# GuildOfWeavers/distaff

Hardware: AMD Instinct MI355X
Metric: trace_cells_per_sec (higher is better)
Workload: dtype u128 (prime field 2^128-45*2^40+1, 4x u32 limbs)

## Files before the change

distaff_amd/csrc/air_kernel.h:

```cpp
#pragma once
#include "ctx.h"
#include <type_traits>

#ifndef AIR_THREADS
#define AIR_THREADS 128
#endif
#ifdef AIR_CONVOY
#define AIR_SYNC() __builtin_amdgcn_s_barrier()
#else
#define AIR_SYNC()
#endif
#ifndef AIR_WAVES_PER_SIMD
#define AIR_WAVES_PER_SIMD 2
#endif
constexpr int air_waves_per_simd(int sd, int slcap, int sect) {
    (void)sd; (void)slcap; (void)sect;
#ifdef AIR_WAVES_FORCE
    return AIR_WAVES_FORCE;
#else
    return AIR_WAVES_PER_SIMD;
#endif
}

struct AirConsts { fe sponge_mds[16], sponge_inv_mds[16], hasher_mds[36], hasher_inv_mds[36]; };
// ... 114 lines not shown
        if constexpr (I == ST_AUX0) return is_bin(o[0]);
        else if constexpr (I == ST_AUX1) return is_bin(o[1]);
        else if constexpr (I == 0) return fe_sub(nw[0], fe_mul(o[0], o[1]));
        else return L(1);
    }
    else if constexpr (OP == 0x0B) {
        if constexpr (I == ST_AUX0) return is_bin(o[0]);
        else if constexpr (I == ST_AUX1) return is_bin(o[1]);
        else if constexpr (I == 0) return fe_sub(nw[0], fe_sub(fe_add(o[0], o[1]), fe_mul(o[0], o[1])));
        else return L(1);
    }
    else if constexpr (OP == 0x0C) { if constexpr (I == 0) return fe_sub(fe_one(), fe_mul(nw[0], o[0])); else return C(); }
    else if constexpr (OP == 0x0D) { if constexpr (I == 0) return fe_add(nw[0], o[0]); else return C(); }
    else if constexpr (OP == 0x0E) {
        if constexpr (I == ST_AUX0) return is_bin(o[0]);
        else if constexpr (I == 0) return fe_sub(nw[0], bnot(o[0]));
        else return C();
    }
    else if constexpr (OP == 0x10) return R(1);
    else if constexpr (OP == 0x11) return R(2);
    else if constexpr (OP == 0x12) { if constexpr (I == 0) return fe_sub(nw[0], o[0]); else return R(1); }
    else if constexpr (OP == 0x13) { if constexpr (I < 2) return fe_sub(nw[i], o[i]); else return R(2); }
    else if constexpr (OP == 0x14) { if constexpr (I < 4) return fe_sub(nw[i], o[i]); else return R(4); }
    else if constexpr (OP == 0x15) { if constexpr (I < 2) return nw[i]; else return R(2); }
    else if constexpr (OP == 0x18) { if constexpr (I == 0) return fe_add(fe_sub(nw[0], o[1]), fe_sub(nw[1], o[0])); else return C(); }
    else if constexpr (OP == 0x19) { if constexpr (I < 4) return fe_sub(nw[i], o[i ^ 2]); else return C(); }
    else if constexpr (OP == 0x1A) return fe_sub(nw[i], o[i ^ 4]);
    else if constexpr (OP == 0x1B) { if constexpr (I < 4) return fe_sub(nw[i], o[(i + 3) & 3]); else return C(); }
    else if constexpr (OP == 0x1C) return fe_sub(nw[i], o[(i + 7) & 7]);
    else if constexpr (OP == 0x1D) {
        if constexpr (I == 0) return is_bin(nw[0]);
        else if constexpr (I == 1) return nw[1];
        else if constexpr (I == 2) return fe_sub(nw[2], fe_double(o[2]));
        else if constexpr (I == 3) return fe_sub(nw[3], fe_add(o[3], fe_mul(nw[0], o[2])));
        else return C();
    }
    else return fe_zero();
}

#define AG_LOW(c, b) (1u << ((c) * 4 + (b)))
#define AG_LOW0 0x00Fu
#define AG_LOW1 0x0F0u
#define AG_PUSH 0x100u
#define AG_CMP 0x200u
#define AG_RESCR 0x400u
#define AG_KEEP 0x800u
#define AG_HIGH 0xF00u
#define AG_DEEP 0x1000u
#define AG_STACK_ALL 0x1FFFu
#define AF_FIRST 1
#define AF_LAST 2
#define AF_EV_IN 4
#define AF_EV_OUT 8

struct StDesc { int kind, j; };
template <int SDK, bool DEEP>
constexpr StDesc st_desc(int op, int I) {
    const bool o4_zero = SDK != 0 && SDK <= 4;
    if (I >= 8) {
        if ((op == 0x0A || op == 0x0B)) return StDesc{5, I == ST_AUX0 ? 100 : 101};
        if ((op == 0x06 || op == 0x07) && o4_zero) return StDesc{0, 0};
        return StDesc{5, -1};
    }
    const int i = I;
    auto diff = [&](int j) { return (SDK != 0 && j >= SDK) ? StDesc{4, 0} : StDesc{1, j}; };
    auto rdiff = [&](int j) { return (SDK != 0 && j >= SDK) ? StDesc{3, 0} : StDesc{2, j}; };
    auto L = [&](int num) { return i + num < 8 ? diff(i + num) : (DEEP ? StDesc{5, -1} : StDesc{3, 0}); };
    auto R = [&](int num) { return diff(i - num < 0 ? 0 : i - num); };
    switch (op) {
        case 0x00: return L(1);
        case 0x01: return L(2);
        case 0x02: return i == 0 ? StDesc{5, -1} : L(2);
        case 0x03: return L(1);
        case 0x04: return L(4);
        case 0x05: return i == 0 ? StDesc{5, -1} : L(2);
        case 0x06: return i < 2 ? (o4_zero ? rdiff(i + 2) : StDesc{5, -1}) : L(4);
        case 0x07: return i < 4 ? (o4_zero ? rdiff(i) : StDesc{5, -1}) : L(2);
        case 0x08: case 0x0B: return i == 0 ? StDesc{5, -1} : L(1);
        case 0x09: case 0x0A: return i == 0 ? StDesc{5, 102} : L(1);
        case 0x0C: case 0x0D: case 0x0E: return i == 0 ? StDesc{5, -1} : diff(i);
        case 0x10: return R(1);
        case 0x11: return R(2);
        case 0x12: return i == 0 ? rdiff(0) : R(1);
        case 0x13: return i < 2 ? rdiff(i) : R(2);
        case 0x14: return i < 4 ? rdiff(i) : R(4);
        case 0x15: return i < 2 ? StDesc{3, 0} : R(2);
        case 0x18: return i == 0 ? StDesc{5, -1} : diff(i);
        case 0x19: return i < 4 ? rdiff(i ^ 2) : diff(i);
        case 0x1A: return rdiff(i ^ 4);
        case 0x1B: return i < 4 ? rdiff((i + 3) & 3) : diff(i);
        case 0x1C: return rdiff((i + 7) & 7);
        case 0x1D: return i == 1 ? StDesc{3, 0} : (i < 4 ? StDesc{5, -1} : diff(i));
        default: return StDesc{0, 0};
    }
}
struct StMerge { int n; int kind[4], j[4], lead[4]; int sgn[4][4]; };
template <int BASE, int I, int SDK, bool DEEP>
constexpr StMerge st_merge() {
    StMerge m{};
    for (int a = 0; a < 4; a++) {
        const StDesc d = st_desc<SDK, DEEP>(BASE + a, I);
        bool has = false;
        switch (a) { case 0: has = st_has<BASE, I>(); break; case 1: has = st_has<BASE + 1, I>(); break; case 2: has = st_has<BASE + 2, I>(); break; default: has = st_has<BASE + 3, I>(); }
        if (!has || d.kind == 0) continue;
        const int cls = d.kind == 5 ? 5 : (d.kind <= 2 ? 1 : 3);
        const int sign = (d.kind == 2 || d.kind == 4) ? -1 : 1;
// ... 54 lines not shown
                constexpr int base = 4 * b + 16 * c;
                if constexpr ((GROUPS & AG_LOW(c, b)) != 0) {
                    static constexpr StMerge M = st_merge<base, I, SDK, DEEP>();
                    if constexpr (M.n > 0) {
                        fe_acc inner; fe_acc_zero(inner);
                        static_for_air<0, M.n>([&](auto e_) {
                            constexpr int e = decltype(e_)::value;
                            fe cf = (base == 0 && M.lead[e] == 0) ? lo0h : lo2[M.lead[e]];
                            static_for_air<0, 4>([&](auto a_) {
                                constexpr int a = decltype(a_)::value;
                                if constexpr (a != M.lead[e] && M.sgn[e][a] != 0) {
                                    const fe other = (base == 0 && a == 0) ? lo0h : lo2[a];
                                    cf = M.sgn[e][a] > 0 ? fe_add(cf, other) : fe_sub(cf, other);
                                }
                            });
                            constexpr int ii = I < 8 ? I : 0;
                            fe term;
                            if constexpr (M.kind[e] == 1) term = fe_sub(s.o[M.j[e]], s.nw[ii]);
                            else if constexpr (M.kind[e] == 2) term = fe_sub(s.nw[ii], s.o[M.j[e]]);
                            else if constexpr (M.kind[e] == 3) term = s.nw[ii];
                            else if constexpr (M.kind[e] == 4) term = fe_neg(s.nw[ii]);
                            else term = st_term<base + M.lead[e], I>(s);
                            fe_acc_mac(inner, cf, term);
                        });
                        fe_acc_mac(middle, mid[b], fe_acc_reduce(inner));
                    }
                }
            });
            fe_acc_mac(outer, top[c], fe_acc_reduce(middle));
        }
    });
    if constexpr ((GROUPS & AG_HIGH) != 0) st_high_degree<I, GROUPS>(outer, s, h);
    return fe_acc_reduce(outer);
}

template <uint32_t ACC_MASK>
struct Acc {
    fe_acc res_acc;
    fe_acc adj_acc[6];
    fe res, adj[6];
    bool nonzero;
    const fe* tc; uint32_t nc;
    __device__ __forceinline__ void emit(uint32_t cidx, int slot, const fe& d) {
        nonzero |= !fe_is_zero(d);
        fe_acc_mac(res_acc, d, tc[cidx]);
        if ((ACC_MASK >> slot) & 1u) fe_acc_mac(adj_acc[slot], d, tc[nc + cidx]);
        else adj[slot] = fe_add(adj[slot], fe_mul(d, tc[nc + cidx]));
    }
};

template <int CL, int LL, int SD, int SLCAP, int SECT, uint32_t GROUPS, int FLAGS>
__global__ void __launch_bounds__(AIR_THREADS, air_waves_per_simd(SD, SLCAP, SECT)) air_kernel(AirArgs a) {
    constexpr bool FIRST = (FLAGS & AF_FIRST) != 0, LAST = (FLAGS & AF_LAST) != 0, EV_IN = (FLAGS & AF_EV_IN) != 0, EV_OUT = (FLAGS & AF_EV_OUT) != 0;
    constexpr int SL = SD ? (SD > 8 ? SD : 8) : SLCAP;
    constexpr bool DEEP = SD == 0 && SLCAP == 12;
    const int cl = (int)a.cl, ll = (int)a.ll;
    const int sl = SD ? SL : (int)a.sl;
    const int sd = SD ? SD : (int)a.stack_depth;
    const fe* c_sponge_mds = a.consts->sponge_mds; const fe* c_sponge_inv_mds = a.consts->sponge_inv_mds;
    const fe* c_hasher_mds = a.consts->hasher_mds; const fe* c_hasher_inv_mds = a.consts->hasher_inv_mds;
    const size_t k = (size_t)blockIdx.x * AIR_THREADS + threadIdx.x;
    if (k >= a.n) return;
    const uint32_t ql = blockIdx.y;
    const uint32_t qg = a.q0 + ql;
    const uint32_t jl = ql * a.coset_step;
    const size_t kn = (k + 1 == a.n) ? 0 : k + 1;
    const fe* cur_p = a.lde + (size_t)jl * a.n + k;
    const fe* nxt_p = a.lde + (size_t)jl * a.n + kn;
    const size_t cs = a.col_stride;
#define CUR(c) cur_p[(size_t)(c) * cs]
#define NXT(c) nxt_p[(size_t)(c) * cs]

    const uint64_t nmask = ((uint64_t)1 << a.log_N) - 1;
    const uint64_t gi = ((uint64_t)k << a.log_b) + (uint64_t)qg * a.coset_step;
    const uint32_t step = (uint32_t)(((uint64_t)k << 3) + qg);
    const uint64_t n64 = a.n;

    const fe c_opc = CUR(0), n_opc = NXT(0);
    fe c_sp[4], n_sp[4], cf[3], ld[5], hd[2], n_cf[3];
#pragma unroll
    for (int i = 0; i < 4; i++) { c_sp[i] = CUR(1 + i); n_sp[i] = NXT(1 + i); }
#pragma unroll
    for (int i = 0; i < 3; i++) { cf[i] = CUR(5 + i); n_cf[i] = NXT(5 + i); }
#pragma unroll
    for (int i = 0; i < 5; i++) ld[i] = CUR(8 + i);
#pragma unroll
    for (int i = 0; i < 2; i++) hd[i] = CUR(13 + i);
    fe c_ctx[CL], n_ctx[CL], c_lp[LL], n_lp[LL], o[SL], nw[SL];
    {
        uint32_t col = 15;
#pragma unroll
        for (int i = 0; i < CL; i++) { bool on = (uint32_t)i < a.ctx_depth; c_ctx[i] = on ? CUR(col + i) : fe_zero(); n_ctx[i] = on ? NXT(col + i) : fe_zero(); }
        col += a.ctx_depth;
#pragma unroll
        for (int i = 0; i < LL; i++) { bool on = (uint32_t)i < a.loop_depth; c_lp[i] = on ? CUR(col + i) : fe_zero(); n_lp[i] = on ? NXT(col + i) : fe_zero(); }
        col += a.loop_depth;
#pragma unroll
        for (int i = 0; i < SL; i++) { bool on = i < sd; o[i] = on ? CUR(col + i) : fe_zero(); nw[i] = on ? NXT(col + i) : fe_zero(); }
    }

    if constexpr ((SECT & 1) != 0) {
        const fe xp = dpow(a, (gi * (6 * n64 + 2)) & nmask);
        const fe one = fe_one();
#pragma unroll 1
        for (int pass = 0; pass < 2; pass++) {
            const fe* cc = a.coef + pass * 94;
            fe_acc R, A; fe_acc_zero(R); fe_acc_zero(A);
            auto term = [&](const fe& v, uint32_t idx) { fe_acc_mac(R, v, cc[idx]); fe_acc_mac(A, v, cc[idx + 1]); };
            term(pass ? fe_sub(c_opc, a.op_count) : c_opc, 0);
            if (pass == 0) { for (int i = 0; i < 4; i++) term(c_sp[i], 2 + 2 * i); }
            else { for (int i = 0; i < 2; i++) term(fe_sub(c_sp[i], a.program_hash[i]), 2 + 2 * i); }
            for (int i = 0; i < 3; i++) term(pass ? fe_sub(cf[i], one) : cf[i], 10 + 2 * i);
            for (int i = 0; i < 5; i++) term(pass ? fe_sub(ld[i], one) : ld[i], 16 + 2 * i);
            for (int i = 0; i < 2; i++) term(pass ? fe_sub(hd[i], one) : hd[i], 26 + 2 * i);
            for (int i = 0; i < CL; i++) if (i < cl) term(c_ctx[i], 30 + 2 * i);
            for (int i = 0; i < LL; i++) if (i < ll) term(c_lp[i], 62 + 2 * i);
            const uint32_t nio = pass ? a.num_outputs : a.num_inputs;
#pragma unroll
            for (int i = 0; i < 8; i++) if ((uint32_t)i < nio) term(fe_sub(o[i], pass ? a.outputs[i] : a.inputs[i]), 78 + 2 * i);
            const fe adj = fe_acc_reduce(A);
            fe_acc_mac(R, adj, xp);
            a.out[((size_t)pass * gridDim.y + ql) * a.n + k] = fe_acc_reduce(R);
        }
    }

    AIR_SYNC();
    fe cff[8], hdf[4], begin_flag, noop_flag, n_void, assert_flag;
    fe lo2[4], mid[4], top[2];
    {
        fe n0 = bnot(cf[0]), n1 = bnot(cf[1]), n2 = bnot(cf[2]);
        fe t0 = fe_mul(n0, n1), t1 = fe_mul(cf[0], n1), t2 = fe_mul(n0, cf[1]), t3 = fe_mul(cf[0], cf[1]);
        cff[0] = fe_mul(t0, n2); cff[1] = fe_mul(t1, n2); cff[2] = fe_mul(t2, n2); cff[3] = fe_mul(t3, n2);
        cff[4] = fe_mul(t0, cf[2]); cff[5] = fe_mul(t1, cf[2]); cff[6] = fe_mul(t2, cf[2]); cff[7] = fe_mul(t3, cf[2]);
        n_void = fe_mul(fe_mul(n_cf[0], n_cf[1]), n_cf[2]);
        fe l0 = bnot(ld[0]), l1 = bnot(ld[1]), l2 = bnot(ld[2]), l3 = bnot(ld[3]);
        lo2[0] = fe_mul(l0, l1); lo2[1] = fe_mul(ld[0], l1);
        lo2[2] = fe_mul(l0, cf[1]);
        lo2[3] = fe_mul(ld[0], ld[1]);
        mid[0] = fe_mul(l2, l3); mid[1] = fe_mul(ld[2], l3); mid[2] = fe_mul(l2, ld[3]); mid[3] = fe_mul(ld[2], ld[3]);
        top[0] = bnot(ld[4]); top[1] = ld[4];
        fe h0 = bnot(hd[0]), h1 = bnot(hd[1]);
        hdf[0] = fe_mul(h0, h1); hdf[1] = fe_mul(hd[0], h1); hdf[2] = fe_mul(h0, hd[1]); hdf[3] = fe_mul(hd[0], hd[1]);
    }
    auto LDF = [&](int idx) { return fe_mul(fe_mul(lo2[idx & 3], mid[(idx >> 2) & 3]), top[idx >> 4]); };
    {
        fe ld0 = LDF(0);
        begin_flag = fe_mul(ld0, hdf[0]);
        noop_flag = fe_mul(LDF(31), hdf[3]);
        hdf[0] = fe_mul(hdf[0], ld[0]);
        assert_flag = fe_mul(ld0, hd[0]);
    }

    AIR_SYNC();
    const fe* per = a.periodic + (size_t)(step & 127u) * AIR_PERIODIC_STRIDE;
    constexpr uint32_t ACC_MASK = !(SD != 0 || SLCAP == 8 || DEEP) ? 0u : ((SECT & 2) ? 0x01u : 0x3Fu);
    Acc<ACC_MASK> acc;
#pragma unroll
    for (int i = 0; i < 6; i++) if ((ACC_MASK >> i) & 1u) fe_acc_zero(acc.adj_acc[i]);
    fe_acc_zero(acc.res_acc); acc.res = fe_zero(); acc.nonzero = false; acc.tc = a.tc; acc.nc = 20 + cl + ll + 2 + sd;
#pragma unroll
    for (int i = 0; i < 6; i++) acc.adj[i] = fe_zero();
    const size_t pstride = (size_t)gridDim.y * a.n, pidx = (size_t)ql * a.n + k;

    if constexpr ((SECT & 2) != 0) {
        fe cf_sum = fe_add(fe_add(cf[0], cf[1]), cf[2]);
        fe ld_prod = fe_mul(fe_mul(fe_mul(ld[0], ld[1]), fe_mul(ld[2], ld[3])), ld[4]);
        fe hd_prod = fe_mul(hd[0], hd[1]);
#pragma unroll
        for (int i = 0; i < 3; i++) acc.emit(i, 0, is_bin(cf[i]));
#pragma unroll
        for (int i = 0; i < 5; i++) acc.emit(3 + i, 0, is_bin(ld[i]));
#pragma unroll
        for (int i = 0; i < 2; i++) acc.emit(8 + i, 0, is_bin(hd[i]));
        const fe is_hacc = cff[0];
        fe hacc_tr = fe_mul(fe_add(c_opc, fe_one()), is_hacc);
        fe rest_tr = fe_mul(c_opc, bnot(is_hacc));
        acc.emit(10, 1, fe_sub(fe_add(hacc_tr, rest_tr), n_opc));
        acc.emit(11, 5, fe_mul(c_opc, fe_mul(bnot(ld_prod), bnot(hd_prod))));
        acc.emit(12, 5, fe_mul(cf_sum, bnot(fe_mul(ld_prod, hd_prod))));
        acc.emit(13, 3, fe_mul(cff[7], bnot(n_void)));
        fe prefix = fe_add(fe_add(cff[1], cff[4]), fe_add(cff[5], cff[6]));
        fe v = fe_mul(prefix, per[21]);
        v = fe_add(v, fe_mul(fe_add(cff[2], cff[3]), per[20]));
        v = fe_add(v, fe_mul(hdf[0], per[22]));
        acc.emit(14, 2, v);
    }

    if constexpr ((SECT & 4) != 0) {
        fe sp[4];
        const fe f_begin = cff[1], f_tend = cff[2], f_fend = cff[3], f_loop = cff[4], f_wrap = cff[5], f_break = cff[6], f_void = cff[7];
        {
            fe os[4], ns[4];
#pragma unroll
            for (int i = 0; i < 4; i++) os[i] = fe_cube(fe_add(c_sp[i], per[i]));
            matmul<4>(os, c_sponge_mds);
            fe op_code = hd[1];
            op_code = fe_add(fe_double(op_code), hd[0]);
            op_code = fe_add(fe_double(op_code), ld[4]);
            op_code = fe_add(fe_double(op_code), ld[3]);
            op_code = fe_add(fe_double(op_code), ld[2]);
            op_code = fe_add(fe_double(op_code), ld[1]);
            op_code = fe_add(fe_double(op_code), ld[0]);
            os[0] = fe_add(os[0], op_code);
            os[1] = fe_add(os[1], fe_mul(nw[0], hdf[0]));
#pragma unroll
            for (int i = 0; i < 4; i++) ns[i] = n_sp[i];
            matmul<4>(ns, c_sponge_inv_mds);
#pragma unroll
            for (int i = 0; i < 4; i++) ns[i] = fe_sub(fe_cube(ns[i]), per[4 + i]);
            const fe clr = fe_add(fe_add(f_begin, f_loop), f_wrap);
            const fe cpy = fe_add(f_break, f_void);
            const fe tf = fe_add(f_tend, f_fend);
            const fe xf[4] = {tf, f_tend, f_fend, tf};
            const fe xv[4] = {fe_sub(c_ctx[0], n_sp[0]), fe_sub(c_sp[0], n_sp[1]), fe_sub(c_sp[0], n_sp[2]), n_sp[3]};
#pragma unroll
            for (int i = 0; i < 4; i++) {
                fe_acc A; fe_acc_zero(A);
                fe_acc_mac(A, cff[0], fe_sub(os[i], ns[i]));
                fe_acc_mac(A, clr, n_sp[i]);
                fe_acc_mac(A, cpy, fe_sub(c_sp[i], n_sp[i]));
                fe_acc_mac(A, xf[i], xv[i]);
                sp[i] = fe_acc_reduce(A);
            }
        }
        acc.emit(15, 3, sp[0]); acc.emit(16, 4, sp[1]); acc.emit(17, 3, sp[2]); acc.emit(18, 3, sp[3]);
    }
    if constexpr ((SECT & 128) != 0) {
        const fe f_begin = cff[1], f_tend = cff[2], f_fend = cff[3], f_loop = cff[4], f_wrap = cff[5], f_break = cff[6], f_void = cff[7];
        acc.emit(19, 2, fe_mul(fe_add(f_wrap, f_break), fe_sub(c_sp[0], c_lp[0])));
        const fe push = fe_add(f_begin, f_loop), pop = fe_add(f_tend, f_fend), ccpy = fe_add(fe_add(f_wrap, f_break), f_void);
        const fe lcpy = fe_add(fe_add(fe_add(f_begin, f_tend), fe_add(f_fend, f_wrap)), f_void);
        if constexpr (CL <= 2 && LL <= 1) {
#pragma unroll
            for (int i = 0; i < CL; i++) {
                if (i >= cl) break;
                fe_acc A; fe_acc_zero(A);
                fe_acc_mac(A, push, fe_sub(i == 0 ? c_sp[0] : c_ctx[i - 1 < 0 ? 0 : i - 1], n_ctx[i]));
                fe_acc_mac(A, pop, i + 1 < cl ? fe_sub(c_ctx[i + 1 < CL ? i + 1 : 0], n_ctx[i]) : n_ctx[i]);
                fe_acc_mac(A, ccpy, fe_sub(c_ctx[i], n_ctx[i]));
                const fe v = fe_acc_reduce(A);
                acc.emit(20 + i, 2, v);
            }
#pragma unroll
            for (int i = 0; i < LL; i++) {
                if (i >= ll) break;
                fe v = fe_mul(lcpy, fe_sub(c_lp[i], n_lp[i]));
                if (i >= 1) v = fe_add(v, fe_mul(f_loop, fe_sub(c_lp[i - 1 < 0 ? 0 : i - 1], n_lp[i])));
                v = fe_add(v, fe_mul(f_break, i + 1 < ll ? fe_sub(c_lp[i + 1 < LL ? i + 1 : 0], n_lp[i]) : n_lp[i]));
                acc.emit(20 + cl + i, 2, v);
            }
        } else {
            auto ctx_cur = [&](int i) { return (uint32_t)i < a.ctx_depth ? CUR(15 + i) : fe_zero(); };
            auto ctx_nxt = [&](int i) { return (uint32_t)i < a.ctx_depth ? NXT(15 + i) : fe_zero(); };
            const uint32_t lcol = 15 + a.ctx_depth;
            auto lp_cur = [&](int i) { return (uint32_t)i < a.loop_depth ? CUR(lcol + i) : fe_zero(); };
            auto lp_nxt = [&](int i) { return (uint32_t)i < a.loop_depth ? NXT(lcol + i) : fe_zero(); };
#pragma unroll 1
            for (int i = 0; i < cl; i++) {
                const fe ni = ctx_nxt(i);
                fe_acc A; fe_acc_zero(A);
                fe_acc_mac(A, push, fe_sub(i == 0 ? c_sp[0] : ctx_cur(i - 1), ni));
                fe_acc_mac(A, pop, i + 1 < cl ? fe_sub(ctx_cur(i + 1), ni) : ni);
                fe_acc_mac(A, ccpy, fe_sub(ctx_cur(i), ni));
                acc.emit(20 + i, 2, fe_acc_reduce(A));
// ... 189 lines not shown
            f = hdf[2];
            fe os[6], ns[6];
#pragma unroll
            for (int i = 0; i < 6; i++) os[i] = fe_cube(fe_add(o[i], per[8 + i]));
            matmul<6>(os, c_hasher_mds);
#pragma unroll
            for (int i = 0; i < 6; i++) ns[i] = nw[i];
            matmul<6>(ns, c_hasher_inv_mds);
#pragma unroll
            for (int i = 0; i < 6; i++) ns[i] = fe_sub(fe_cube(ns[i]), per[14 + i]);
#pragma unroll
            for (int i = 0; i < 6; i++) agg(i, f, fe_sub(ns[i], os[i]));
            copy_from(6, f);
        }
        }

        const uint32_t sbase = 20 + cl + ll;
        if constexpr ((SECT & 40) != 0) { acc.emit(sbase, 4, aux0); acc.emit(sbase + 1, 4, aux1); }
#pragma unroll
        for (int i = 0; i < SLR; i++) if (i < sd) acc.emit(sbase + 2 + i, 4, ev[i]);
    }
    if constexpr (DEEP && (GROUPS & AG_DEEP) != 0) {
        {
            const uint32_t sbase = 20 + cl + ll;
            const fe lo_all = fe_add(fe_add(lo2[0], lo2[1]), fe_add(lo2[2], lo2[3]));
            fe fl1, fl2, fl4, fr1, fr2, fr4, fcp;
            { fe_acc A; fe_acc_zero(A); fe_acc_mac(A, mid[0], lo2[3]); fe_acc_mac(A, mid[2], lo_all); fl1 = fe_add(fe_mul(top[0], fe_acc_reduce(A)), assert_flag); }
            { fe_acc A; fe_acc_zero(A); fe_acc_mac(A, mid[0], fe_add(lo2[1], lo2[2])); fe_acc_mac(A, mid[1], fe_add(lo2[1], lo2[3])); fl2 = fe_mul(top[0], fe_acc_reduce(A)); }
            fl4 = fe_mul(top[0], fe_mul(mid[1], fe_add(lo2[0], lo2[2])));
            fr1 = fe_add(fe_mul(top[1], fe_mul(mid[0], fe_add(lo2[0], lo2[2]))), hdf[0]);
            { fe_acc A; fe_acc_zero(A); fe_acc_mac(A, mid[0], fe_add(lo2[1], lo2[3])); fe_acc_mac(A, mid[1], lo2[1]); fr2 = fe_mul(top[1], fe_acc_reduce(A)); }
            fr4 = fe_mul(top[1], fe_mul(mid[1], lo2[0]));
            {
                fe_acc A; fe_acc_zero(A); fe_acc_mac(A, mid[2], lo_all); fe_acc_mac(A, mid[3], fe_add(lo2[0], lo2[1]));
                fe_acc B; fe_acc_zero(B); fe_acc_mac(B, top[1], fe_acc_reduce(A)); fe_acc_mac(B, top[0], fe_mul(mid[3], fe_add(fe_add(lo2[0], lo2[1]), lo2[2])));
                fcp = fe_add(fe_add(fe_acc_reduce(B), fe_add(hdf[1], hdf[2])), fe_add(begin_flag, noop_flag));
            }
            const uint32_t scol = 15 + a.ctx_depth + a.loop_depth;
#pragma unroll 1
            for (int i = 8; i < sd; i++) {
                const fe ni = NXT(scol + i);
                auto item = [&](int j) { return CUR(scol + j); };
                auto left = [&](int num) { return i + num < sl ? fe_sub(item(i + num), ni) : ni; };
                fe_acc A; fe_acc_zero(A);
                fe_acc_mac(A, fcp, fe_sub(item(i), ni));
                fe_acc_mac(A, fr1, fe_sub(item(i - 1), ni)); fe_acc_mac(A, fr2, fe_sub(item(i - 2), ni)); fe_acc_mac(A, fr4, fe_sub(item(i - 4), ni));
                fe_acc_mac(A, fl1, left(1)); fe_acc_mac(A, fl2, left(2)); fe_acc_mac(A, fl4, left(4));
                acc.emit(sbase + 2 + i, 4, fe_acc_reduce(A));
            }
        }
    }

    if constexpr (SECT == 1) return;
    const bool on_trace = (qg == 0);
    if (on_trace && k + 1 != a.n && acc.nonzero) atomicMin(a.bad_step, (unsigned long long)k);
    acc.res = fe_acc_reduce(acc.res_acc);
    constexpr bool EMITS_STACK = (SECT & 120) != 0 || (GROUPS & AG_DEEP) != 0 || ((GROUPS & AG_STACK_ALL) != 0 && !EV_OUT);
    constexpr uint32_t USED = ((SECT & 2) ? 0x2Fu : 0u) | ((SECT & 4) ? 0x18u : 0u) | ((SECT & 128) ? 0x04u : 0u) | (EMITS_STACK ? 0x10u : 0u);
#pragma unroll
    for (int i = 0; i < 6; i++) if (((ACC_MASK & USED) >> i) & 1u) acc.adj[i] = fe_add(acc.adj[i], fe_acc_reduce(acc.adj_acc[i]));
    if constexpr (!FIRST) {
        acc.res = fe_add(acc.res, a.partial[pidx]);
#pragma unroll
        for (int i = 0; i < 6; i++) if (LAST || ((USED >> i) & 1u)) acc.adj[i] = fe_add(acc.adj[i], a.partial[(size_t)(i + 1) * pstride + pidx]);
    }
    if constexpr (!LAST) {
        a.partial[pidx] = acc.res;
#pragma unroll
        for (int i = 0; i < 6; i++) if (FIRST || ((USED >> i) & 1u)) a.partial[(size_t)(i + 1) * pstride + pidx] = acc.adj[i];
        return;
    }
    fe t;
    if (on_trace && k + 1 != a.n) {
        t = fe_zero();
    } else {
        const uint32_t degs[6] = {2, 3, 4, 6, 7, 8};
        fe_acc T; fe_acc_zero(T);
        fe_acc_add(T, acc.res);
#pragma unroll
        for (int g = 0; g < 6; g++) {
            uint64_t p = 8 * n64 - 1 - (n64 - 1) * degs[g];
            fe_acc_mac(T, acc.adj[g], dpow(a, (gi * p) & nmask));
        }
        t = fe_acc_reduce(T);
    }
    a.out[((size_t)2 * gridDim.y + ql) * a.n + k] = t;
#undef CUR
#undef NXT
}


template <int CL, int LL, int SD, int SLCAP, int SECT, uint32_t GROUPS, int FLAGS>
static void launch_air(dst_ctx* c, const AirArgs& a, uint32_t Q) {
    dim3 g((unsigned)((c->n + AIR_THREADS - 1) / AIR_THREADS), Q);
    static char name[64];
    if (!name[0]) snprintf(name, sizeof(name), "air_kernel<%d,%d,%d,%d,%d,%u,%d>", CL, LL, SD, SLCAP, SECT, (unsigned)GROUPS, FLAGS);
    constexpr int NS = SD == 4 ? 6 : 10;
    const double units = c->W + ((FLAGS & AF_FIRST) ? 0 : 7) + ((FLAGS & AF_LAST) ? 1 : 7) + ((SECT & 1) ? 2 : 0) + ((FLAGS & AF_EV_IN) ? NS : 0) + ((FLAGS & AF_EV_OUT) ? NS : 0);
    { KScope ks_(c, name, 16.0 * c->n * Q * units, true); hipLaunchKernelGGL((air_kernel<CL, LL, SD, SLCAP, SECT, GROUPS, FLAGS>), g, dim3(AIR_THREADS), 0, c->stream, a); }
}
void air_launch_sd4(dst_ctx* c, const AirArgs& a, uint32_t Q);
void air_launch_small(dst_ctx* c, const AirArgs& a, uint32_t Q);
void air_launch_deep(dst_ctx* c, const AirArgs& a, uint32_t Q);
void air_launch_generic(dst_ctx* c, const AirArgs& a, uint32_t Q);
```

distaff_amd/csrc/ctx.h:

```cpp
#pragma once
#include <hip/hip_runtime.h>
#include <stdint.h>
#include <string.h>
#include <memory>
#include <string>
#include <map>
#include <vector>
#include "fe.h"
#include "../../include/distaff_hip.h"

struct __attribute__((aligned(16))) digest { uint32_t w[8]; };
#define AIR_PERIODIC_STRIDE 29

#ifndef NTT_TW4_PAIRS
#define NTT_TW4_PAIRS 0
#endif
#if NTT_TW4_PAIRS
typedef fe_tw tw4_t;
#else
typedef fe tw4_t;
#endif

#define DST_MAX_FRI_LAYERS 24

struct dst_switch_def { const char* name; bool product; const char* values; const char* what; };
static const dst_switch_def DST_SWITCHES[] = {
    {"DISTAFF_SHARD_DEBUG",        true,  "1",               "stderr line per tree exchange on rank 0; communicators record the order of their collectives (dst_comm_trace)"},
    {"DISTAFF_SHARD_TREE_GATHER",  true,  "1",               "sharded Merkle trees: all-gather of all boundary nodes + upper levels repeated on every rank (BASELINE north_star's all-gather-only form) instead of the k-range all-to-all"},
    {"DISTAFF_SHARD_NO_OVERLAP",   true,  "1",               "sharded prover: every collective on the context's main stream (no second stream / events) also on a stream-ordered transport"},
    {"DISTAFF_COMM_TIMEOUT_S",     true,  "seconds",         "communicators: limit of every host wait behind a collective (default 60; <= 0: none); on expiry the rank aborts the communicator and returns DST_ERR_COMM (dst_comm_set_timeout changes it per handle)"},
    {"DISTAFF_LOCAL_TRANSPORT",    true,  "blocking",        "in-process transport (dst_comm_init_local, dst_prove_sharded_local): drain every rank's stream around each collective instead of the stream-ordered form (events between the ranks' streams, nothing waited for)"},
    {"DISTAFF_TMP_REGS",           true,  "4..W",            "registers per transform launch = size of the staging array (default: as many as 12 GiB hold, at most W)"},
    {"DISTAFF_AIR",                false, "small|deep|generic", "force a more general constraint-kernel instance set than the trace shape needs (generic = per-operation formulation)"},
    {"DISTAFF_BOUNDARY",           false, "eval",            "boundary combinations by evaluation on the 8n domain (the reference's route) instead of coefficient form"},
    {"DISTAFF_COMBINE",            false, "steps",           "combine_polys / DEEP composition as the reference's sequence of whole-array steps instead of the fused passes"},
    {"DISTAFF_NTT",                false, "pre|3pass|reg|lds", "force a transform plan family"},
    {"DISTAFF_NTT_SHAPE",          false, "a,b",             "three-pass plans: log2 of the first two pass lengths"},
    {"DISTAFF_NTT_ORDER",          false, "0",               "first pass of an extension in coset-slow block order"},
    {"DISTAFF_NTT_WAVES",          false, "4|8",             "force the 512- or 1024-lane instances of the LDS passes"},
    {"DISTAFF_NTT_FIXED",          false, "0",               "use the any-shape instances where a shape-compiled one exists"},
    {"DISTAFF_NTT_DIF",            false, "0|1|2",           "first pass of an extension: coset DIT (0), pre-scale + DIF (1), DIT with last-stage twiddles from global memory (2)"},
    {"DISTAFF_NTT_DEBUG",          false, "1",               "print the occupancy of every transform launch shape once"},
    {"DISTAFF_LDE_BATCH",          false, "cols,cosets",     "registers x cosets per transform launch"},
    {"DISTAFF_FOLD8_DFT",          false, "0",               "8n-coefficient extensions without the fused fold + 8-point step"},
    {"DISTAFF_TRACE_BUFFER",       false, "1",               "give the trace its own buffer instead of coset 0 of the extension"},
    {"DISTAFF_MERKLE_LEVEL2_LOG",  false, "k",               "build two tree levels per launch from 2^k grandparents per launch on (default 2^19)"},
    {"DISTAFF_MERKLE_LEVELS",      false, "1",               "one launch per tree level"},
    {"DISTAFF_SYN_DIV_TABLES",     false, "1",               "synthetic division by power tables + scan instead of the blocked form"},
    {"DISTAFF_FRI_TAIL",           false, "0",               "no single-launch tail: every FRI layer by its own launches (the tail otherwise starts at the first layer of at most 2^13 elements)"},
    {"DISTAFF_FRI_CHAIN",          false, "0",               "FRI commit phase with a root read-back and a host draw per layer"},
    {"DISTAFF_FRI_REPLICATE_LOG",  false, "k",               "sharded prover: replicate FRI layers from 2^k elements on (default 2^17)"},
    {"DISTAFF_SHARD_FORCE_OVERLAP", false, "1",              "sharded prover: the two-stream choreography of a stream-ordered transport over a blocking one"},
    {"DISTAFF_TEST_STALL_COLLECTIVE", false, "k|k@r",        "communicators: fault injection -- before device collective number k (of rank r only) a kernel holds the stream until the communicator is aborted"},
};
enum : size_t {
    HS_WEIGHTS = 0,
    HS_WEIGHTS_BYTES = (4 * 128 + 4) * 16,
    HS_DEEP = 32768,
    HS_DEEP_HALF = 2048,
    HS_FRI_ROOTS = 40960,
    HS_FRI_SLOTS = 45056,
    HS_FRI_SLOT_BYTES = 800,
    HS_AIR_FLAG = 65536 - 64,
    HS_DRAWS = 65536,
    HS_DRAWS_BYTES = (344 + 160) * 16,
    HS_COMPOSE = 65536 + 8192,
    HS_COMPOSE_BYTES = 516 * 16,
    HS_STATUS = 65536 + 8192 + 8320,
    HS_STATUS_SLOTS = 32,
    HS_TREE_READBACK = 65536 + 8192 + 8320 + 2048,
    HS_TAIL_ROOTS = HS_TREE_READBACK + 1024,
    HS_POW = HS_TAIL_ROOTS + 1024,
    HS_TOTAL = 131072
};
static_assert(HS_WEIGHTS + HS_WEIGHTS_BYTES <= HS_DEEP, "boundary weights overlap the DEEP values");
static_assert(HS_DEEP_HALF >= 128 * 16 && HS_DEEP + 2 * HS_DEEP_HALF <= HS_FRI_ROOTS, "DEEP values: W <= 128 registers");
static_assert(HS_FRI_ROOTS + DST_MAX_FRI_LAYERS * 32 <= HS_FRI_SLOTS, "FRI roots overlap the layer slots");
static_assert(8 * 96 + 32 <= HS_FRI_SLOT_BYTES && HS_FRI_SLOTS + DST_MAX_FRI_LAYERS * HS_FRI_SLOT_BYTES <= HS_AIR_FLAG, "FRI layer slots: G <= 8 ranks, DST_MAX_FRI_LAYERS layers");
static_assert(HS_DRAWS + HS_DRAWS_BYTES <= HS_COMPOSE && HS_COMPOSE + HS_COMPOSE_BYTES <= HS_STATUS && HS_STATUS + HS_STATUS_SLOTS * 64 <= HS_TOTAL, "upload regions overlap");
static_assert(HS_STATUS_SLOTS >= 2 + DST_MAX_FRI_LAYERS, "one status slot per tree exchange of a proof");
static_assert(HS_STATUS + HS_STATUS_SLOTS * 64 <= HS_TREE_READBACK && 8 * 96 + 32 <= 1024 && DST_MAX_FRI_LAYERS * 32 <= 1024 && HS_POW + 64 <= HS_TOTAL, "read-back regions overlap");

#ifdef DISTAFF_TEST_HOOKS
#define DST_TEST_HOOKS 1
#else
#define DST_TEST_HOOKS 0
// ... 124 lines not shown
    bool have_trace = false, committed = false, constraints_done = false, composed = false;
    hipStream_t upload_stream = nullptr;
    std::vector<hipEvent_t> upload_done;
    std::vector<size_t> upload_bounds;
    bool upload_pending = false;
    bool trace_owned_only = false;
    bool ceval_inverted = false;
    hipStream_t comm_stream = nullptr;
    std::vector<hipEvent_t> comm_events;
    uint8_t* d_status = nullptr;
    double phase_ms[9] = {0};
    double shard_ms[2] = {0, 0};
    uint32_t shard_trees = 0;
    struct dst_comm* wait_comm = nullptr;
    hipEvent_t sh_ev[8] = {nullptr};
    struct CollEv { hipEvent_t e0, e1; int kind; };
    std::vector<CollEv> coll_ev;
    size_t coll_used = 0;
    double exchange_ms[8] = {0};

    int profile = 0;
    struct KEvent { hipEvent_t e0, e1; std::string name; double bytes, mads; };
    std::vector<KEvent> kpending;
    std::vector<hipEvent_t> event_pool;
    struct KStat { uint64_t launches = 0; double ms = 0, bytes = 0, mads = 0; };
    std::map<std::string, KStat> kstats;
};

struct KScope {
    dst_ctx* c; bool on;
    dst_ctx::KEvent ev;
    KScope(dst_ctx* ctx, const char* name, double bytes, bool heavy = false, double mads = 0.0) : c(ctx), on(ctx->profile == 1 || (ctx->profile == 2 && heavy)) {
        if (!on) return;
        ev.name = name; ev.bytes = bytes; ev.mads = mads;
        if (c->event_pool.size() >= 2) { ev.e0 = c->event_pool.back(); c->event_pool.pop_back(); ev.e1 = c->event_pool.back(); c->event_pool.pop_back(); }
        else if (hipEventCreate(&ev.e0) != hipSuccess || hipEventCreate(&ev.e1) != hipSuccess) { on = false; return; }
        (void)hipEventRecord(ev.e0, c->stream);
    }
    ~KScope() { if (on) { (void)hipEventRecord(ev.e1, c->stream); c->kpending.push_back(ev); } }
};

#define HIP_TRY(ctx, expr)                                                                          \
    do {                                                                                            \
        hipError_t _e = (expr);                                                                     \
        if (_e != hipSuccess) {                                                                     \
            (ctx)->err = std::string(#expr) + ": " + hipGetErrorString(_e);                          \
            return DST_ERR_HIP;                                                                     \
        }                                                                                           \
    } while (0)

int ctx_sync(dst_ctx* c, const char* what);
#define CTX_SYNC(ctx, what) do { const int _r = ctx_sync((ctx), (what)); if (_r) return _r; } while (0)

inline bool dst_internal_boundary_by_evaluation(const dst_ctx* c) { return DST_TEST_HOOKS && c->sw_is("DISTAFF_BOUNDARY", "eval"); }
inline bool dst_internal_combine_by_steps(const dst_ctx* c) { return DST_TEST_HOOKS && (c->sw_is("DISTAFF_COMBINE", "steps") || dst_internal_boundary_by_evaluation(c)); }
inline bool fri_tail_starts_at(const dst_ctx* c, int d) {
    if (d < 1 || d >= c->num_fri_layers || c->fri_size[d] > ((size_t)1 << 13)) return false;
    const char* e = c->sw("DISTAFF_FRI_TAIL");
    return !(e && e[0] == '0');
}
int k_ntt_init(dst_ctx* c);
void k_intt_columns(dst_ctx* c, const fe* src, size_t src_stride, fe* dst, size_t ncols);
void k_lde_columns(dst_ctx* c, const fe* polys, fe* lde, size_t ncols);
void k_lde_fold8(dst_ctx* c, const fe* poly8n, fe* out);
void k_intt8_cosets(dst_ctx* c, fe* vals , fe* out8n, fe* work);
void k_coset_to_natural_len(dst_ctx* c, const fe* src, size_t cosets, size_t len, fe* dst);
void k_fri_leaves_at(dst_ctx* c, const fe* e, digest* leaves, size_t R);
void k_fri_fold_at(dst_ctx* c, const fe* e, fe* out, size_t R, int layer, fe special_x, const fe* alpha_dev = nullptr);
void k_trace_leaves(dst_ctx* c);
void k_merkle(dst_ctx* c, const digest* leaves, digest* nodes, size_t count, size_t stop_count);
void k_constraint_tree(dst_ctx* c);
void k_fri_leaves_layer0(dst_ctx* c);
void k_fri_leaves(dst_ctx* c, int layer);
int k_eval_constraints(dst_ctx* c, const fe* coeffs_dev, const fe* tc_dev, int64_t* bad_step, bool defer_check = false);
int k_constraint_check(dst_ctx* c, int64_t* bad_step);
void k_syn_div(dst_ctx* c, fe* a, size_t len, fe b);
void k_syn_div_batch(dst_ctx* c, fe* const* a, const fe* b, int count, size_t len);
void k_syn_div_compose(dst_ctx* c, const fe* a, fe* out, size_t len, fe b, const fe* t, size_t tn, size_t inc, fe k1, fe k2, fe k3);
void k_combine_fused(dst_ctx* c, const fe* work, const fe* q4, size_t q_stride, fe* cpoly);
void k_syn_div_expanded(dst_ctx* c, const fe* a, fe* out, size_t len, size_t degree, fe exception);
void k_horner(dst_ctx* c, const fe* polys, size_t ncols, size_t len, fe x, fe* out_dev);
void k_lincomb(dst_ctx* c, const fe* cols, size_t ncols, size_t len, const fe* coeffs_dev, fe* out);
void k_lincomb2(dst_ctx* c, const fe* cols, size_t ncols, size_t len, const fe* coeffs_dev, size_t coef_stride, fe* out0, fe* out1);
void k_lincomb4(dst_ctx* c, const fe* cols, size_t ncols, size_t len, const fe* coeffs_dev, fe* out0, fe* out1, fe* out2, fe* out3);
void k_axpy(dst_ctx* c, fe* y, const fe* x, fe a, size_t len);
void k_add(dst_ctx* c, fe* y, const fe* x, size_t len);
void k_sub_dot_at0(dst_ctx* c, fe* y, const fe* values_dev, const fe* coeffs_dev, size_t count);
void k_sub_at0(dst_ctx* c, fe* y, const fe* v_dev);
void k_fri_fold(dst_ctx* c, int layer, fe special_x);
void k_fri_fold_dev(dst_ctx* c, int layer, const fe* alpha_dev);
void k_fri_draw(dst_ctx* c, int layer, fe* alpha_out, digest* root_out);
void k_intt_cosets_local(dst_ctx* c, fe* vals, fe* out, size_t cosets);
void k_cross8(dst_ctx* c, const fe* work, fe* out8n);
int k_fri_tail(dst_ctx* c, int first, uint8_t* roots_out);
int k_pow(dst_ctx* c, const uint8_t seed[32], uint32_t grinding, uint64_t* nonce);
void k_gather(dst_ctx* c, const void* src, size_t item_bytes, const uint64_t* idx_dev, size_t count, void* dst);
void k_gather_rows(dst_ctx* c, const uint64_t* positions_dev, size_t count, fe* out);
void k_gather_pieces(dst_ctx* c, const uint64_t* addr_dev, size_t count, void* dst);
int k_bench_mulmod(dst_ctx* c, uint64_t lanes, uint32_t iters, double* ms);
int k_bench_mad(dst_ctx* c, uint64_t lanes, uint32_t iters, double* ms);
int k_bench_clock(dst_ctx* c, uint64_t lanes, uint32_t iters, double* mhz);
int k_bench_code(dst_ctx* c, uint32_t code_kib, double* ms);
void k_upper_tree(dst_ctx* c, const digest* gathered, digest* upper, size_t nb, uint32_t G);
void k_digests_from_records(dst_ctx* c, const void* recs, size_t stride, digest* dst, size_t count);
void k_constraint_level1(dst_ctx* c);
void k_fri_leaves_cm(dst_ctx* c, const fe* e, digest* leaves, size_t nd);
// ... 13 lines not shown
```

distaff_amd/csrc/kernels_air_deep.hip:

```cpp
#include "air_kernel.h"
void air_launch_deep(dst_ctx* c, const AirArgs& a, uint32_t Q) {
#if DST_TEST_HOOKS
    if (dst_internal_boundary_by_evaluation(c)) launch_air<16, 8, 0, 12, 1, 0, 0>(c, a, Q);
#endif
    launch_air<16, 8, 0, 12, 2, 0, AF_FIRST>(c, a, Q);
    launch_air<16, 8, 0, 12, 4, 0, 0>(c, a, Q);
    launch_air<16, 8, 0, 12, 128, 0, 0>(c, a, Q);
    launch_air<16, 8, 0, 12, 0, AG_DEEP, 0>(c, a, Q);
    launch_air<16, 8, 0, 12, 0, AG_RESCR, AF_EV_OUT>(c, a, Q);
    launch_air<16, 8, 0, 12, 0, AG_PUSH | AG_CMP | AG_KEEP, AF_EV_IN | AF_EV_OUT>(c, a, Q);
    launch_air<16, 8, 0, 12, 0, AG_LOW(0, 0) | AG_LOW(0, 2), AF_EV_IN | AF_EV_OUT>(c, a, Q);
    launch_air<16, 8, 0, 12, 0, AG_LOW(0, 1) | AG_LOW(0, 3), AF_EV_IN | AF_EV_OUT>(c, a, Q);
    launch_air<16, 8, 0, 12, 0, AG_LOW(1, 2) | AG_LOW(1, 3), AF_EV_IN | AF_EV_OUT>(c, a, Q);
    launch_air<16, 8, 0, 12, 0, AG_LOW(1, 0) | AG_LOW(1, 1), AF_EV_IN | AF_LAST>(c, a, Q);
}
```

distaff_amd/csrc/kernels_air_sd4.hip:

```cpp
#include "air_kernel.h"
void air_launch_sd4(dst_ctx* c, const AirArgs& a, uint32_t Q) {
#if DST_TEST_HOOKS
    if (dst_internal_boundary_by_evaluation(c)) launch_air<2, 1, 4, 8, 1, 0, 0>(c, a, Q);
#endif
    launch_air<2, 1, 4, 8, 130, 0, AF_FIRST>(c, a, Q);
    launch_air<2, 1, 4, 8, 4, 0, 0>(c, a, Q);
    launch_air<2, 1, 4, 8, 0, AG_HIGH, AF_EV_OUT>(c, a, Q);
    launch_air<2, 1, 4, 8, 0, AG_LOW0, AF_EV_IN | AF_EV_OUT>(c, a, Q);
    launch_air<2, 1, 4, 8, 0, AG_LOW1, AF_EV_IN | AF_LAST>(c, a, Q);
}
```

distaff_amd/csrc/kernels_air_small.hip:

```cpp
#include "air_kernel.h"
void air_launch_small(dst_ctx* c, const AirArgs& a, uint32_t Q) {
#if DST_TEST_HOOKS
    if (dst_internal_boundary_by_evaluation(c)) launch_air<2, 1, 0, 8, 1, 0, 0>(c, a, Q);
#endif
    launch_air<2, 1, 0, 8, 130, 0, AF_FIRST>(c, a, Q);
    launch_air<2, 1, 0, 8, 4, 0, 0>(c, a, Q);
    launch_air<2, 1, 0, 8, 0, AG_RESCR, AF_EV_OUT>(c, a, Q);
    launch_air<2, 1, 0, 8, 0, AG_PUSH | AG_CMP | AG_KEEP, AF_EV_IN | AF_EV_OUT>(c, a, Q);
    launch_air<2, 1, 0, 8, 0, AG_LOW(0, 0) | AG_LOW(0, 2), AF_EV_IN | AF_EV_OUT>(c, a, Q);
    launch_air<2, 1, 0, 8, 0, AG_LOW(0, 1) | AG_LOW(0, 3), AF_EV_IN | AF_EV_OUT>(c, a, Q);
    launch_air<2, 1, 0, 8, 0, AG_LOW(1, 2) | AG_LOW(1, 3), AF_EV_IN | AF_EV_OUT>(c, a, Q);
    launch_air<2, 1, 0, 8, 0, AG_LOW(1, 0) | AG_LOW(1, 1), AF_EV_IN | AF_LAST>(c, a, Q);
}
```

Measured before the change: 599.9 million.

## Hand operation flags from the op-bit launch to the sponge launch via buffers

The launch that evaluates op-bit constraints now stores six derived flag products (cff[0], sponge clear/copy sums, cff[2], cff[3], hdf[0]) into the ev scratch arrays. The sponge-section launch then loads them instead of recomputing the field-multiply flag tree. This trades several 128-bit modular multiplies per cell for six extra global stores and loads per cell. It also adds an early return for launches that use no accumulator slots, which skips the bad-step check and the reductions.

```diff
diff --git a/distaff_amd/csrc/air_kernel.h b/distaff_amd/csrc/air_kernel.h
--- a/distaff_amd/csrc/air_kernel.h
+++ b/distaff_amd/csrc/air_kernel.h
@@ -190,6 +190,8 @@
 #define AF_LAST 2
 #define AF_EV_IN 4
 #define AF_EV_OUT 8
+#define AF_FL_OUT 16
+#define AF_FL_IN 32
 
 struct StDesc { int kind, j; };
 template <int SDK, bool DEEP>
@@ -350,6 +352,9 @@
 template <int CL, int LL, int SD, int SLCAP, int SECT, uint32_t GROUPS, int FLAGS>
 __global__ void __launch_bounds__(AIR_THREADS, air_waves_per_simd(SD, SLCAP, SECT)) air_kernel(AirArgs a) {
     constexpr bool FIRST = (FLAGS & AF_FIRST) != 0, LAST = (FLAGS & AF_LAST) != 0, EV_IN = (FLAGS & AF_EV_IN) != 0, EV_OUT = (FLAGS & AF_EV_OUT) != 0;
+    constexpr bool FL_OUT = (FLAGS & AF_FL_OUT) != 0, FL_IN = (FLAGS & AF_FL_IN) != 0;
+    static_assert(!FL_OUT || (SECT & 2) != 0, "the launch that hands the sponge's flags on is the one with the op bits: it forms all of them anyway");
+    static_assert(!FL_IN || (SECT == 4 && GROUPS == 0), "only the sponge section runs on handed-on flags");
     constexpr int SL = SD ? (SD > 8 ? SD : 8) : SLCAP;
     constexpr bool DEEP = SD == 0 && SLCAP == 12;
     const int cl = (int)a.cl, ll = (int)a.ll;
@@ -425,7 +430,11 @@
     AIR_SYNC();
     fe cff[8], hdf[4], begin_flag, noop_flag, n_void, assert_flag;
     fe lo2[4], mid[4], top[2];
-    {
+    fe sp_clr, sp_cpy;
+    const size_t pstride = (size_t)gridDim.y * a.n, pidx = (size_t)ql * a.n + k;
+    if constexpr (FL_IN) {
+        cff[0] = a.ev[0][pidx]; sp_clr = a.ev[1][pidx]; sp_cpy = a.ev[2][pidx]; cff[2] = a.ev[3][pidx]; cff[3] = a.ev[4][pidx]; hdf[0] = a.ev[5][pidx];
+    } else {
         fe n0 = bnot(cf[0]), n1 = bnot(cf[1]), n2 = bnot(cf[2]);
         fe t0 = fe_mul(n0, n1), t1 = fe_mul(cf[0], n1), t2 = fe_mul(n0, cf[1]), t3 = fe_mul(cf[0], cf[1]);
         cff[0] = fe_mul(t0, n2); cff[1] = fe_mul(t1, n2); cff[2] = fe_mul(t2, n2); cff[3] = fe_mul(t3, n2);
@@ -441,12 +450,17 @@
         hdf[0] = fe_mul(h0, h1); hdf[1] = fe_mul(hd[0], h1); hdf[2] = fe_mul(h0, hd[1]); hdf[3] = fe_mul(hd[0], hd[1]);
     }
     auto LDF = [&](int idx) { return fe_mul(fe_mul(lo2[idx & 3], mid[(idx >> 2) & 3]), top[idx >> 4]); };
-    {
+    if constexpr (!FL_IN) {
         fe ld0 = LDF(0);
         begin_flag = fe_mul(ld0, hdf[0]);
         noop_flag = fe_mul(LDF(31), hdf[3]);
         hdf[0] = fe_mul(hdf[0], ld[0]);
         assert_flag = fe_mul(ld0, hd[0]);
+        sp_clr = fe_add(fe_add(cff[1], cff[4]), cff[5]);
+        sp_cpy = fe_add(cff[6], cff[7]);
+    }
+    if constexpr (FL_OUT) {
+        a.ev[0][pidx] = cff[0]; a.ev[1][pidx] = sp_clr; a.ev[2][pidx] = sp_cpy; a.ev[3][pidx] = cff[2]; a.ev[4][pidx] = cff[3]; a.ev[5][pidx] = hdf[0];
     }
 
     AIR_SYNC();
@@ -458,7 +472,6 @@
     fe_acc_zero(acc.res_acc); acc.res = fe_zero(); acc.nonzero = false; acc.tc = a.tc; acc.nc = 20 + cl + ll + 2 + sd;
 #pragma unroll
     for (int i = 0; i < 6; i++) acc.adj[i] = fe_zero();
-    const size_t pstride = (size_t)gridDim.y * a.n, pidx = (size_t)ql * a.n + k;
 
     if constexpr ((SECT & 2) != 0) {
         fe cf_sum = fe_add(fe_add(cf[0], cf[1]), cf[2]);
@@ -486,7 +499,7 @@
 
     if constexpr ((SECT & 4) != 0) {
         fe sp[4];
-        const fe f_begin = cff[1], f_tend = cff[2], f_fend = cff[3], f_loop = cff[4], f_wrap = cff[5], f_break = cff[6], f_void = cff[7];
+        const fe f_tend = cff[2], f_fend = cff[3];
         {
             fe os[4], ns[4];
 #pragma unroll
@@ -506,8 +519,7 @@
             matmul<4>(ns, c_sponge_inv_mds);
 #pragma unroll
             for (int i = 0; i < 4; i++) ns[i] = fe_sub(fe_cube(ns[i]), per[4 + i]);
-            const fe clr = fe_add(fe_add(f_begin, f_loop), f_wrap);
-            const fe cpy = fe_add(f_break, f_void);
+            const fe clr = sp_clr, cpy = sp_cpy;
             const fe tf = fe_add(f_tend, f_fend);
             const fe xf[4] = {tf, f_tend, f_fend, tf};
             const fe xv[4] = {fe_sub(c_ctx[0], n_sp[0]), fe_sub(c_sp[0], n_sp[1]), fe_sub(c_sp[0], n_sp[2]), n_sp[3]};
@@ -803,11 +815,12 @@
     }
 
     if constexpr (SECT == 1) return;
+    constexpr bool EMITS_STACK = (SECT & 120) != 0 || (GROUPS & AG_DEEP) != 0 || ((GROUPS & AG_STACK_ALL) != 0 && !EV_OUT);
+    constexpr uint32_t USED = ((SECT & 2) ? 0x2Fu : 0u) | ((SECT & 4) ? 0x18u : 0u) | ((SECT & 128) ? 0x04u : 0u) | (EMITS_STACK ? 0x10u : 0u);
+    if constexpr (USED == 0 && !FIRST && !LAST) return;
     const bool on_trace = (qg == 0);
     if (on_trace && k + 1 != a.n && acc.nonzero) atomicMin(a.bad_step, (unsigned long long)k);
     acc.res = fe_acc_reduce(acc.res_acc);
-    constexpr bool EMITS_STACK = (SECT & 120) != 0 || (GROUPS & AG_DEEP) != 0 || ((GROUPS & AG_STACK_ALL) != 0 && !EV_OUT);
-    constexpr uint32_t USED = ((SECT & 2) ? 0x2Fu : 0u) | ((SECT & 4) ? 0x18u : 0u) | ((SECT & 128) ? 0x04u : 0u) | (EMITS_STACK ? 0x10u : 0u);
 #pragma unroll
     for (int i = 0; i < 6; i++) if (((ACC_MASK & USED) >> i) & 1u) acc.adj[i] = fe_add(acc.adj[i], fe_acc_reduce(acc.adj_acc[i]));
     if constexpr (!FIRST) {
@@ -847,7 +860,9 @@
     static char name[64];
     if (!name[0]) snprintf(name, sizeof(name), "air_kernel<%d,%d,%d,%d,%d,%u,%d>", CL, LL, SD, SLCAP, SECT, (unsigned)GROUPS, FLAGS);
     constexpr int NS = SD == 4 ? 6 : 10;
-    const double units = c->W + ((FLAGS & AF_FIRST) ? 0 : 7) + ((FLAGS & AF_LAST) ? 1 : 7) + ((SECT & 1) ? 2 : 0) + ((FLAGS & AF_EV_IN) ? NS : 0) + ((FLAGS & AF_EV_OUT) ? NS : 0);
+    constexpr bool IDLE = (SECT & ~1) == 0 && (GROUPS & AG_DEEP) == 0 && (FLAGS & (AF_EV_OUT | AF_FIRST | AF_LAST)) == AF_EV_OUT;
+    const double units = c->W + (((FLAGS & AF_FIRST) || IDLE) ? 0 : 7) + ((FLAGS & AF_LAST) ? 1 : (IDLE ? 0 : 7)) + ((SECT & 1) ? 2 : 0) + ((FLAGS & AF_EV_IN) ? NS : 0) + ((FLAGS & AF_EV_OUT) ? NS : 0)
+                       + ((FLAGS & AF_FL_OUT) ? 6 : 0) + ((FLAGS & AF_FL_IN) ? 6 : 0);
     { KScope ks_(c, name, 16.0 * c->n * Q * units, true); hipLaunchKernelGGL((air_kernel<CL, LL, SD, SLCAP, SECT, GROUPS, FLAGS>), g, dim3(AIR_THREADS), 0, c->stream, a); }
 }
 void air_launch_sd4(dst_ctx* c, const AirArgs& a, uint32_t Q);
diff --git a/distaff_amd/csrc/ctx.h b/distaff_amd/csrc/ctx.h
--- a/distaff_amd/csrc/ctx.h
+++ b/distaff_amd/csrc/ctx.h
@@ -32,6 +32,7 @@
     {"DISTAFF_LOCAL_TRANSPORT",    true,  "blocking",        "in-process transport (dst_comm_init_local, dst_prove_sharded_local): drain every rank's stream around each collective instead of the stream-ordered form (events between the ranks' streams, nothing waited for)"},
     {"DISTAFF_TMP_REGS",           true,  "4..W",            "registers per transform launch = size of the staging array (default: as many as 12 GiB hold, at most W)"},
     {"DISTAFF_AIR",                false, "small|deep|generic", "force a more general constraint-kernel instance set than the trace shape needs (generic = per-operation formulation)"},
+    {"DISTAFF_AIR_HANDOFF",        false, "0",               "constraint launches derive every operation flag they need from the op bits themselves instead of loading those an earlier launch of the evaluation stored"},
     {"DISTAFF_BOUNDARY",           false, "eval",            "boundary combinations by evaluation on the 8n domain (the reference's route) instead of coefficient form"},
     {"DISTAFF_COMBINE",            false, "steps",           "combine_polys / DEEP composition as the reference's sequence of whole-array steps instead of the fused passes"},
     {"DISTAFF_NTT",                false, "pre|3pass|reg|lds", "force a transform plan family"},
@@ -262,6 +263,7 @@
 int ctx_sync(dst_ctx* c, const char* what);
 #define CTX_SYNC(ctx, what) do { const int _r = ctx_sync((ctx), (what)); if (_r) return _r; } while (0)
 
+inline bool dst_internal_air_handoff(const dst_ctx* c) { return !(DST_TEST_HOOKS && c->sw_is("DISTAFF_AIR_HANDOFF", "0")); }
 inline bool dst_internal_boundary_by_evaluation(const dst_ctx* c) { return DST_TEST_HOOKS && c->sw_is("DISTAFF_BOUNDARY", "eval"); }
 inline bool dst_internal_combine_by_steps(const dst_ctx* c) { return DST_TEST_HOOKS && (c->sw_is("DISTAFF_COMBINE", "steps") || dst_internal_boundary_by_evaluation(c)); }
 inline bool fri_tail_starts_at(const dst_ctx* c, int d) {
diff --git a/distaff_amd/csrc/kernels_air_deep.hip b/distaff_amd/csrc/kernels_air_deep.hip
--- a/distaff_amd/csrc/kernels_air_deep.hip
+++ b/distaff_amd/csrc/kernels_air_deep.hip
@@ -3,8 +3,16 @@
 #if DST_TEST_HOOKS
     if (dst_internal_boundary_by_evaluation(c)) launch_air<16, 8, 0, 12, 1, 0, 0>(c, a, Q);
 #endif
-    launch_air<16, 8, 0, 12, 2, 0, AF_FIRST>(c, a, Q);
-    launch_air<16, 8, 0, 12, 4, 0, 0>(c, a, Q);
+    if (dst_internal_air_handoff(c)) {
+        launch_air<16, 8, 0, 12, 2, 0, AF_FIRST | AF_FL_OUT>(c, a, Q);
+        launch_air<16, 8, 0, 12, 4, 0, AF_FL_IN>(c, a, Q);
+    }
+#if DST_TEST_HOOKS
+    else {
+        launch_air<16, 8, 0, 12, 2, 0, AF_FIRST>(c, a, Q);
+        launch_air<16, 8, 0, 12, 4, 0, 0>(c, a, Q);
+    }
+#endif
     launch_air<16, 8, 0, 12, 128, 0, 0>(c, a, Q);
     launch_air<16, 8, 0, 12, 0, AG_DEEP, 0>(c, a, Q);
     launch_air<16, 8, 0, 12, 0, AG_RESCR, AF_EV_OUT>(c, a, Q);
diff --git a/distaff_amd/csrc/kernels_air_sd4.hip b/distaff_amd/csrc/kernels_air_sd4.hip
--- a/distaff_amd/csrc/kernels_air_sd4.hip
+++ b/distaff_amd/csrc/kernels_air_sd4.hip
@@ -3,8 +3,16 @@
 #if DST_TEST_HOOKS
     if (dst_internal_boundary_by_evaluation(c)) launch_air<2, 1, 4, 8, 1, 0, 0>(c, a, Q);
 #endif
-    launch_air<2, 1, 4, 8, 130, 0, AF_FIRST>(c, a, Q);
-    launch_air<2, 1, 4, 8, 4, 0, 0>(c, a, Q);
+    if (dst_internal_air_handoff(c)) {
+        launch_air<2, 1, 4, 8, 130, 0, AF_FIRST | AF_FL_OUT>(c, a, Q);
+        launch_air<2, 1, 4, 8, 4, 0, AF_FL_IN>(c, a, Q);
+    }
+#if DST_TEST_HOOKS
+    else {
+        launch_air<2, 1, 4, 8, 130, 0, AF_FIRST>(c, a, Q);
+        launch_air<2, 1, 4, 8, 4, 0, 0>(c, a, Q);
+    }
+#endif
     launch_air<2, 1, 4, 8, 0, AG_HIGH, AF_EV_OUT>(c, a, Q);
     launch_air<2, 1, 4, 8, 0, AG_LOW0, AF_EV_IN | AF_EV_OUT>(c, a, Q);
     launch_air<2, 1, 4, 8, 0, AG_LOW1, AF_EV_IN | AF_LAST>(c, a, Q);
diff --git a/distaff_amd/csrc/kernels_air_small.hip b/distaff_amd/csrc/kernels_air_small.hip
--- a/distaff_amd/csrc/kernels_air_small.hip
+++ b/distaff_amd/csrc/kernels_air_small.hip
@@ -3,8 +3,16 @@
 #if DST_TEST_HOOKS
     if (dst_internal_boundary_by_evaluation(c)) launch_air<2, 1, 0, 8, 1, 0, 0>(c, a, Q);
 #endif
-    launch_air<2, 1, 0, 8, 130, 0, AF_FIRST>(c, a, Q);
-    launch_air<2, 1, 0, 8, 4, 0, 0>(c, a, Q);
+    if (dst_internal_air_handoff(c)) {
+        launch_air<2, 1, 0, 8, 130, 0, AF_FIRST | AF_FL_OUT>(c, a, Q);
+        launch_air<2, 1, 0, 8, 4, 0, AF_FL_IN>(c, a, Q);
+    }
+#if DST_TEST_HOOKS
+    else {
+        launch_air<2, 1, 0, 8, 130, 0, AF_FIRST>(c, a, Q);
+        launch_air<2, 1, 0, 8, 4, 0, 0>(c, a, Q);
+    }
+#endif
     launch_air<2, 1, 0, 8, 0, AG_RESCR, AF_EV_OUT>(c, a, Q);
     launch_air<2, 1, 0, 8, 0, AG_PUSH | AG_CMP | AG_KEEP, AF_EV_IN | AF_EV_OUT>(c, a, Q);
     launch_air<2, 1, 0, 8, 0, AG_LOW(0, 0) | AG_LOW(0, 2), AF_EV_IN | AF_EV_OUT>(c, a, Q);
```

Measured after the change: 601.0 million, median of 3. About the same (+0.2%).
